# sleveque/control

Measured on AMD Instinct MI355X. Metric: Krylov iterations/s (preconditioned GMRES(10), all-at-once heat-control KKT), higher is better.
Workload: dtype f64; 1 GPU; 2-D heat control, 256^2 P1, n_t=64, beta=0.0001, T=2, BE, mode G; unknowns=8454272, krylov=gmres, left preconditioning, restart 10, classical Gram-Schmidt, parallelism=time-block rows over 1 GPU(s), transport=none, sweep_tiles=boxes from the dof coordinates (kkt_set_tile_coordinates)

## Files before the change

control_amd/_lib.py:

```python
from __future__ import annotations

import ctypes as C
import os

import numpy as np

_HERE = os.path.dirname(os.path.abspath(__file__))
LIB_PATH = os.environ.get("KKT_LIB") or os.path.join(_HERE, "libkkt.so")

c_i32p = C.POINTER(C.c_int32)
c_f64p = C.POINTER(C.c_double)


class KktError(RuntimeError):
    def __init__(self, code, msg):
        super().__init__(f"libkkt error {code}: {msg}")
        self.code = code


class PcDesc(C.Structure):
    _fields_ = [("kind", C.c_int), ("n_t", C.c_int), ("tau", C.c_double),
                ("beta", C.c_double), ("epsilon", C.c_double), ("nx", C.c_int64),
                ("m_indptr", c_i32p), ("m_indices", c_i32p), ("m_values", c_f64p),
                ("n_bc", C.c_int64), ("bc_idx", c_i32p),
# ... 54 lines not shown
    def as_dict(self):
        return {n: getattr(self, n) for n, _ in self._fields_}


class CoarseStats(C.Structure):
    _fields_ = ([(n, C.c_int64) for n in ("matrices", "launches", "n_coarse")] + [("ms", C.c_double)]
                + [(n, C.c_int64) for n in ("blocks", "block_n")])

    def as_dict(self):
        return {n: getattr(self, n) for n, _ in self._fields_}


class SpectrumStats(C.Structure):
    _fields_ = ([(n, C.c_int64) for n in ("matrices", "batches", "lanczos_steps", "power_steps", "launches",
                                          "syncs", "twin_syncs", "lanczos_syncs_max", "fallbacks",
                                          "batch_bytes")] + [("ms", C.c_double)])

    def as_dict(self):
        return {n: getattr(self, n) for n, _ in self._fields_}


class StepLock(C.Structure):
    _fields_ = [("n_steps", C.c_int), ("restart", C.c_int), ("V", c_f64p), ("h", c_f64p),
                ("v_next", c_f64p)]


class RelinDesc(C.Structure):
    _fields_ = ([("n_t", C.c_int), ("cn", C.c_int), ("nq", C.c_int),
                 ("ne", C.c_int64), ("n2", C.c_int64), ("n1", C.c_int64),
                 ("nu", C.c_double), ("tau", C.c_double), ("beta", C.c_double),
                 ("V", c_i32p)] + [(n, c_f64p) for n in ("W", "phi", "gphi", "lam", "glam")]
# ... 186 lines not shown
    "kkt_debug_coarse_inverses": (C.c_int, [C.c_void_p, c_f64p, C.c_int64]),
    "kkt_debug_dense_inverse": (C.c_int, [C.c_void_p, C.c_int, C.c_int, c_f64p, c_f64p, c_i32p]),
    "kkt_debug_coarse_correction": (C.c_int, [C.c_void_p, C.c_int, C.c_int, C.c_int64, c_f64p, c_f64p,
                                              c_f64p, c_f64p, c_f64p, c_f64p, c_i32p]),
    "kkt_debug_krylov_op": (C.c_int, [C.c_void_p, C.c_int, C.c_int64, C.c_int, c_f64p, c_f64p,
                                      c_f64p, C.c_double, C.c_double, c_f64p, c_f64p, c_f64p]),
    "kkt_debug_block_op": (C.c_int, [C.c_void_p, C.POINTER(BlockOp)]),
    "kkt_debug_spectrum_op": (C.c_int, [C.c_void_p, C.POINTER(SpectrumOp)]),
    "kkt_debug_row_step": (C.c_int, [C.c_void_p, C.POINTER(RowStep)]),
    "kkt_debug_tile_levels": (C.c_int, [C.c_void_p, C.POINTER(TileLevels)]),
    "kkt_debug_set_steplock": (C.c_int, [C.c_void_p, C.POINTER(StepLock)]),
    "kkt_debug_apply_forms": (C.c_int, [C.c_void_p, c_i32p, C.c_int]),
    "kkt_debug_pc_forms": (C.c_int, [C.c_void_p, c_i32p, C.c_int]),
    "kkt_debug_pc_solves": (C.c_int, [C.c_void_p, c_f64p, C.c_int]),
    "kkt_debug_pc_matrices": (C.c_int, [C.c_void_p, c_f64p, C.c_int]),
    "kkt_debug_mass_tile_values": (C.c_int, [C.c_void_p, C.POINTER(C.c_int64), C.POINTER(C.c_int64),
                                             c_f64p, c_i32p, c_f64p]),
    "kkt_get_info": (C.c_int, [C.c_void_p, C.POINTER(Info)]),
    "kkt_comm_unique_id": (C.c_int, [C.c_void_p]),
    "kkt_comm_init_rccl": (C.c_int, [C.c_void_p, C.c_void_p]),
    "kkt_comm_init_callbacks": (C.c_int, [C.c_void_p, ALLREDUCE_FN, SENDRECV_FN,
                                          C.c_void_p]),
    "kkt_comm_barrier": (C.c_int, [C.c_void_p]),
    "kkt_comm_max": (C.c_int, [C.c_void_p, c_f64p]),
}

_lib = None


def load():
# ... 25 lines not shown
```

control_amd/csrc/capi.cpp:

```cpp
#include <algorithm>
#include <charconv>
#include <climits>
#include <cmath>
#include <cstring>
#include <string>

#include "comm.hpp"
#include "pc.hpp"
#include "reaction.hpp"
#include "relin.hpp"
#include "system.hpp"
#include "tiles.hpp"

using namespace kkt;

struct kkt_system {
    System S;
};

static std::string g_create_error;

#define KKT_TRY(h, ...)                                   \
    if (!(h)) return KKT_ERR_ARG;                         \
    System &S = (h)->S;                                   \
// ... 74 lines not shown
    {"no_graph", "0 | 1", set_switch<&Options::no_graph>},
    {"persistent", "0 | 1", set_switch<&Options::persistent>},
    {"prog_mode", "auto | tile | dataflow | flags | w", set_prog_mode},
    {"prog_waves", "1..8", set_int<&Options::prog_waves, 1, 8>},
    {"prog_steps", "0 | 1", set_switch<&Options::prog_steps>},
    {"tile_depth", "1..16", set_int<&Options::tile_depth, 1, TILE_MAX_DEPTH>},
    {"tile_waves", "1..16", set_int<&Options::tile_waves, 1, 16>},
    {"tile_unfused", "0 | 1", set_switch<&Options::tile_unfused>},
    {"tile_poll_delay", "an integer", set_int<&Options::tile_poll_delay>},
    {"lanes", "0 | 1", set_switch<&Options::lanes>},
    {"lane_chunks", "an integer", set_int<&Options::lane_chunks>},
    {"coarse_setup", "batched | columns", set_coarse_setup},
    {"coarse_keep", "0 | 1", set_switch<&Options::coarse_keep>},
    {"coarse_blocks", "0 | 1", set_switch<&Options::coarse_blocks>},
    {"spectrum_batch", "0..4096", set_int<&Options::spectrum_batch, 0, 4096>},
    {"coarse_rings", "0 | 1", set_switch<&Options::coarse_rings>},
    {"tile_coarse_cache", "auto | 0 | 1 | 2", set_tile_coarse_cache},
    {"tile_coarse_rows", "block | full", set_tile_coarse_rows},
    {"mass_tiles", "0 | 1", set_switch<&Options::mass_tiles>},
    {"mass_tile_depth", "0..8", set_int<&Options::mass_tile_depth, 0, MASS_TILE_MAX_DEPTH>},
    {"mass_tile_rows", "0..65536", set_int<&Options::mass_tile_rows, 0, 65536>},
    {"mass_tile_levels", "0..4096", set_int<&Options::mass_tile_levels, 0, 4096>},
    {"mass_tile_waves", "0 | 4 | 8", set_mass_tile_waves},
    {"stage_timers", "0 | 1", set_switch<&Options::stage_timers>},
    {"verbose", "0 | 1", set_switch<&Options::verbose>},
    {"stamps", "0 | 1", set_switch<&Options::stamps>},
    {"debug_drop_handoff", "an integer", set_int<&Options::debug_drop_handoff>},
};

extern "C" {
// ... 481 lines not shown
            const bool grouped = L.ngroups > 0 && rowops_grouped_kernel(L.R, L.uniform_w);
            rec.insert(rec.end(), {L.R, L.uniform_w, grouped ? L.ngroups : 0, sorted});
        }
        return put_forms(rec, KKT_APPLY_FORM_INTS, out, cap);
    });
}

int kkt_debug_pc_forms(kkt_handle h, int32_t *out, int cap) {
    KKT_TRY(h, {
        std::vector<int32_t> rec;
        if (S.pc) S.pc->plain_forms(rec);
        return put_forms(rec, KKT_PC_FORM_INTS, out, cap);
    });
}

static int put_records(const std::vector<double> &rec, int per, double *out, int cap) {
    const int n = (int)rec.size() / per;
    if (out) {
        if (cap < (int)rec.size()) fail(KKT_ERR_ARG, "buffer too small for the records");
        std::copy(rec.begin(), rec.end(), out);
    }
    return n;
}

int kkt_debug_pc_solves(kkt_handle h, double *out, int cap) {
    KKT_TRY(h, {
        std::vector<double> rec;
        if (S.pc) S.pc->solve_records(rec);
        return put_records(rec, KKT_PC_SOLVE_VALS, out, cap);
    });
// ... 71 lines not shown
```

control_amd/csrc/pc.cpp:

```cpp
#include "pc.hpp"

#include <algorithm>
#include <chrono>
#include <cmath>
#include <cstdlib>
#include <cstdio>
#include <cstring>

namespace kkt {

SchurPC::SchurPC(System &S, const kkt_pc_desc &d) : S_(S), d_(d) {
    if (!S.finalized) fail(KKT_ERR_STATE, "kkt_set_pc_schur needs a finalized system");
    if (d.kind < KKT_PC_STATIONARY || d.kind > KKT_PC_INSTATIONARY_CN)
        fail(KKT_ERR_ARG, "unknown preconditioner kind");
    if (!d.m_indptr || !d.m_indices || !d.m_values) fail(KKT_ERR_ARG, "mass matrix missing");
    if (S.nx0 != S.nx1 || d.nx != S.nx0)
        fail(KKT_ERR_ARG, "built-in preconditioner needs equal spatial spaces of size nx");
    nx_ = d.nx;
    if (d.kind == KKT_PC_STATIONARY)
        n_ = 1;
    else
        n_ = d.kind == KKT_PC_INSTATIONARY_BE ? d.n_t : d.n_t - 1;
    if (n_ != S.n0 || n_ != S.n1 || n_ < 1)
        fail(KKT_ERR_ARG, "n_t does not match the block counts of the system");
// ... 63 lines not shown

void SchurPC::emit_wait(int lane, int ev) {
    PcStep s;
    s.kind = PcStep::EV_WAIT;
    s.lane = lane;
    s.ev = ev;
    steps_.push_back(s);
}

void SchurPC::values_changed() {
    clear_program();
    values_mem_.release();
    mats_.clear();
    mat_recs_.clear();
    solve_recs_.clear();
    einvs_.clear();
    pending_coarse_.clear();
    S_.spectrum_stats = kkt_spectrum_stats{};
    collect_matrices();
    if (d_.kind == KKT_PC_STATIONARY)
        build_stationary();
    else if (d_.kind == KKT_PC_INSTATIONARY_BE)
        build_BE();
    else
        build_CN();
    pre_.clear();
    pre_cls_.clear();
    flush_coarse();
    if (S_.opts.verbose && d_.schur_emin <= 0) {
        std::fprintf(stderr, "[kkt] Chebyshev sub-solves: degree %d; %lld Lanczos steps spent on "
// ... 400 lines not shown
        return out;
    }
    const bool be = d_.kind == KKT_PC_INSTATIONARY_BE;
    const double shift = d_.tau / std::sqrt(d_.beta);
    auto coef = [&](int i) {
        if (!be) return 0.5 * d_.tau / std::sqrt(d_.beta);
        return i == 0 ? 0.0 : (i == n - 1 ? std::sqrt(d_.epsilon) * shift : shift);
    };
    const int imid = (lo + hi) / 2;
    out.emplace_back(block_vals(KKT_Q10, imid, imid), coef(imid));
    for (int i = lo; i < hi; ++i) out.emplace_back(block_vals(KKT_Q10, i, i), coef(i));
    for (int i = hi - 1; i >= lo; --i) out.emplace_back(block_vals(KKT_Q01, i, i), coef(i));
    return out;
}

void SchurPC::collect_matrices() {
    pre_.clear();
    pre_cls_.clear();
    const int nbatch = S_.opts.spectrum_batch;
    const bool estimates = d_.schur_emin <= 0;
    if (nbatch <= 0 || !(estimates || coarse_cycles_ > 0)) return;
    const Pattern &P = S_.patterns[m_pat_];
    hipStream_t st = S_.stream;
    kkt_spectrum_stats &stats = S_.spectrum_stats;
    SpectrumCounters cnt;
    HIPCHK(hipStreamSynchronize(st));
    const auto t0 = std::chrono::steady_clock::now();
    std::vector<MatKey> keys;
    for (const auto &bc : solved_matrices()) {
        uint64_t bits;
        std::memcpy(&bits, &bc.second, sizeof bits);
        const MatKey key(bc.first, bits);
        if (pre_.count(key)) continue;
        Pre pr;
        pr.vals = values_mem_.alloc<double>(P.npadded);
        pr.dinv = values_mem_.alloc<double>(nx_);
        form_matrix(bc.first, bc.second, pr.vals, pr.dinv);
        cnt.launches += mask_ ? 3 : 2;
        pre_[key] = pr;
        keys.push_back(key);
    }
    const int C = (int)keys.size();
    if (C == 0) return;
    spec::TwinGroups twins;
    twins.first_of.resize(C);
    for (int i = 0; i < C; ++i) twins.first_of[i] = i;
    twins.pair_of.assign(C, -1);
    std::vector<unsigned> h_flag;
    DevPool tmp;
    if (C > 1) {
        std::vector<const double *> h_vals(C);
        for (int i = 0; i < C; ++i) h_vals[i] = pre_[keys[i]].vals;
        const double *const *d_vals = tmp.upload(h_vals.data(), h_vals.size());
        const int nw = spec_fingerprint_blocks(P.npadded);
        unsigned long long *d_fp = tmp.alloc<unsigned long long>((size_t)C * nw);
        std::vector<unsigned long long> h_fp((size_t)C * nw);
        launch_spec_fingerprint(st, d_vals, C, P.npadded, d_fp);
        HIPCHK(hipGetLastError());
        HIPCHK(hipMemcpyAsync(h_fp.data(), d_fp, h_fp.size() * sizeof(unsigned long long),
                              hipMemcpyDeviceToHost, st));
        HIPCHK(hipStreamSynchronize(st));
        cnt.launches++;
        cnt.syncs++;
        stats.twin_syncs++;
        std::vector<uint64_t> shifts(C), folded(C);
        for (int i = 0; i < C; ++i) {
            shifts[i] = keys[i].second;
            folded[i] = spec_fingerprint_fold(&h_fp[(size_t)i * nw], nw);
        }
        twins = spec::group_twins(shifts, folded);
        std::vector<SpecPair> pairs;
        for (const auto &pr : twins.pairs) pairs.push_back(SpecPair{h_vals[pr.first], h_vals[pr.second]});
        if (!pairs.empty()) {
            const SpecPair *d_pairs = tmp.upload(pairs.data(), pairs.size());
            unsigned *d_flag = tmp.alloc<unsigned>(pairs.size());
            h_flag.assign(pairs.size(), 1u);
            HIPCHK(hipMemsetAsync(d_flag, 0, pairs.size() * sizeof(unsigned), st));
            launch_spec_pairs_differ(st, d_pairs, (int)pairs.size(), P.npadded, d_flag);
            HIPCHK(hipGetLastError());
            HIPCHK(hipMemcpyAsync(h_flag.data(), d_flag, h_flag.size() * sizeof(unsigned),
                                  hipMemcpyDeviceToHost, st));
            HIPCHK(hipStreamSynchronize(st));
            cnt.launches++;
            cnt.syncs++;
            stats.twin_syncs++;
        }
    }
    std::vector<int> reps;
    const std::vector<int> cls = spec::twin_classes(twins, h_flag, &reps);
    for (int i = 0; i < C; ++i) pre_[keys[i]].cls = cls[i];
    pre_cls_.assign(reps.size(), PreCls{});
    const int32_t *tpos = estimates ? transpose_positions() : nullptr;
    for (size_t r0 = 0; estimates && r0 < reps.size(); r0 += (size_t)nbatch) {
        const int B = (int)std::min<size_t>((size_t)nbatch, reps.size() - r0);
        DevPool bmem;
        std::vector<const double *> lv(B), dv(B);
        std::vector<SpecSplit> split(B);
        std::vector<unsigned> nonsym(B, 0u);
        for (int b = 0; b < B; ++b) {
            const Pre &pr = pre_[keys[reps[r0 + b]]];
            lv[b] = pr.vals;
            dv[b] = pr.dinv;
        }
        size_t split_bytes = 0;
        if (tpos) {
            for (int b = 0; b < B; ++b)
// ... 59 lines not shown
    std::memcpy(&bits, &c, sizeof bits);
    auto key = std::make_pair(base_vals, bits);
    auto it = mats_.find(key);
    if (it != mats_.end() && (!solved || it->second.est != KKT_PC_EST_NONE)) return it->second;
    const Pattern &P = S_.patterns[m_pat_];
    hipStream_t st = S_.stream;
    Mat m;
    if (it != mats_.end()) {
        m = it->second;
    } else {
        const auto pre = pre_.find(key);
        if (pre != pre_.end()) {
            m.vals = pre->second.vals;
            m.dinv = pre->second.dinv;
        } else {
            m.vals = values_mem_.alloc<double>(P.npadded);
            m.dinv = values_mem_.alloc<double>(nx_);
            form_matrix(base_vals, c, m.vals, m.dinv);
        }
        m.index = (int)mat_recs_.size();
        MatRec r;
        r.c = c;
        mat_recs_.push_back(r);
    }
    if (!solved) {
        mats_[key] = m;
        return m;
    }
    MatRec &rec = mat_recs_[m.index];
    const Mat *twin = nullptr;
    kkt_spectrum_stats &stats = S_.spectrum_stats;
    const bool batched = S_.opts.spectrum_batch > 0;
    auto cls_of = [&](const MatKey &k) {
// ... 15 lines not shown
            fell_back = batched;
            stats.launches++;
            stats.syncs++;
            stats.twin_syncs++;
            auto d_flag = DevBuf<unsigned>::alloc(1);
            HIPCHK(hipMemsetAsync(d_flag.get(), 0, sizeof(unsigned), st));
            launch_vals_differ(st, m.vals, kv.second.vals, P.npadded, d_flag.get());
            unsigned differ = 1;
            HIPCHK(hipMemcpyAsync(&differ, d_flag.get(), sizeof differ, hipMemcpyDeviceToHost, st));
            HIPCHK(hipStreamSynchronize(st));
            if (!differ) {
                twin = &kv.second;
                break;
            }
        }
    }
    if (d_.schur_emin > 0) {
        m.emin = d_.schur_emin;
        m.emax = d_.schur_emax;
        m.eimag = d_.schur_eimag > 0 ? d_.schur_eimag : 0.0;
        m.est = KKT_PC_EST_GIVEN;
    } else if (twin) {
        m.emin = twin->emin;
        m.emax = twin->emax;
        m.eimag = twin->eimag;
        m.est = KKT_PC_EST_SHARED;
    } else {
        DevBuf<double> hv, sv2;
        unsigned nonsym = 0;
        Spectrum sp{0.0, 0.0, 0};
// ... 38 lines not shown
            rec.power = power;
        }
        if (coarse_cycles_ > 0) m.emin = std::max(m.emin, m.emax / 30.0);
        m.est = KKT_PC_EST_LANCZOS;
    }
    if (fell_back) stats.fallbacks++;
    if (!batched || fell_back)
        stats.ms += std::chrono::duration<double, std::milli>(std::chrono::steady_clock::now() - t0).count();
    if (coarse_cycles_ > 0) m.einv = twin && twin->einv ? twin->einv : coarse_inverse(m.vals);
    rec.est = m.est;
    rec.coarse = m.einv != nullptr;
    mats_[key] = m;
    return m;
}

void SchurPC::note_solve(int sweep, int level, const Mat &m) {
    mat_recs_[m.index].solves++;
    solve_recs_.insert(solve_recs_.end(),
                       {(double)sweep, (double)level, (double)m.index, mat_recs_[m.index].c, m.emin,
                        m.emax, m.eimag, (double)schur_its_, (double)m.est});
}

void SchurPC::solve_records(std::vector<double> &out) const { out = solve_recs_; }
bool SchurPC::coarse_space(CoarseDev *c, GalerkinDev *g, int64_t *n) const {
    if (coarse_.nc <= 0) return false;
    *c = coarse_;
    *g = galerkin_;
    *n = nx_;
    return true;
}

// ... 192 lines not shown
    if (record_solo) {
        solo.its = its;
        solo.lev = level_form(nullptr, sv[0], scale).lev;
        solo.eligible = true;
        end_level(std::move(solo));
    }
}

void SchurPC::build_stationary() {
    const double c = 1.0 / std::sqrt(d_.beta);
    const double *Dv = block_vals(KKT_Q10, 0, 0);
    const double *Dz = block_vals(KKT_Q01, 0, 0);
    double *b0 = in_, *b1 = in_ + nx_;
    double *u0 = out_, *u1 = out_ + nx_;
    emit_solves({Solve{m_vals_, m_dinv_, b0, u0}}, d_.mass_its, d_.mass_emin, d_.mass_emax, P_, nx_);
    emit_lin({Lin{{Term{Dv, u0}}, B_, 1.0, 0.0, -1.0, nullptr, b1}});
    Mat S1 = schur_matrix(Dv, c), S2 = schur_matrix(Dz, c);
    schur_its_ = resolve_its(S1);
    note_solve(KKT_PC_SWEEP_FIRST, 0, S1);
    emit_solves({Solve{S1.vals, S1.dinv, B_, u1}}, schur_its_, S1.emin, S1.emax, P_, nx_, false, nullptr, S1.eimag, &S1);
    emit_lin({Lin{{Term{m_vals_, u1}}, B_, 1.0}});
    note_solve(KKT_PC_SWEEP_SECOND, 0, S2);
    emit_solves({Solve{S2.vals, S2.dinv, B_, u1}}, schur_its_, S2.emin, S2.emax, P_, nx_, false, nullptr, S2.eimag, &S2);
}


void SchurPC::build_BE() {
    const int n = n_, lo = lo_, hi = hi_;
    const double tau = d_.tau, eps = d_.epsilon;
    const double shift = tau / std::sqrt(d_.beta);
    const int64_t nl = hi - lo;
// ... 16 lines not shown
        const int c0 = cfirst[c], c1 = cfirst[c + 1];
        cur_lane_ = lanes ? 1 : 0;
        {
            std::vector<Solve> sv;
            for (int i = c0; i < c1; ++i)
                sv.push_back(Solve{m_vals_, m_dinv_, blk(b0, i), blk(u0, i), 1.0 / tau,
                                   i == n - 1 ? 1.0 / eps : 1.0});
            double *const Pc[3] = {blk(P_[0], c0), blk(P_[1], c0), blk(P_[2], c0)};
            emit_solves(sv, d_.mass_its, d_.mass_emin, d_.mass_emax, Pc, nx_);
        }
        if (c == n_chunks - 1 && (up >= 0 || dn >= 0)) emit_comm(blk(u0, hi - 1), up, h_u0_, dn);
        {
            std::vector<Lin> ops;
            for (int i = c0; i < c1; ++i) {
                Lin l;
                l.terms.push_back(Term{block_vals(KKT_Q10, i, i), blk(u0, i)});
                if (i >= 1)
                    l.terms.push_back(Term{block_vals(KKT_Q10, i, i - 1),
                                           i - 1 >= lo ? blk(u0, i - 1) : h_u0_});
                l.y = blk(B_, i);
                l.cz = -1.0;
                l.z = blk(b1, i);
                ops.push_back(l);
            }
            emit_lin(ops);
        }
        if (lanes) chunk_done[c] = emit_record(1);
        cur_lane_ = 0;
    };
    auto sweep_chunk = [&](int c) {
        if (lanes) emit_wait(0, chunk_done[c]);
        for (int i = cfirst[c]; i < cfirst[c + 1]; ++i) {
            Mat F = schur_matrix(block_vals(KKT_Q10, i, i), coef(i));
            note_solve(KKT_PC_SWEEP_FORWARD, i, F);
            const Solve sv{F.vals, F.dinv, blk(B_, i), blk(u1, i)};
            if (i >= 1)
                emit_update_and_solve(Lin{{Term{block_vals(KKT_Q10, i, i - 1),
                                                i - 1 >= lo ? blk(u1, i - 1) : h_u1_}},
                                          blk(B_, i), -1.0, 1.0, 0.0, blk(B_, i), nullptr},
                                      sv, schur_its_, F.emin, F.emax, F.eimag, &F);
            else
                emit_solves({sv}, schur_its_, F.emin, F.emax, P_, nx_, false, nullptr, F.eimag, &F);
        }
    };
    if (lanes) {
        const int e_start = emit_record(0);
        emit_wait(1, e_start);
        side_chunk(0);
        for (int c = 0; c < n_chunks; ++c) {
            sweep_chunk(c);
            if (c + 1 < n_chunks) side_chunk(c + 1);
        }
    } else {
        side_chunk(0);
        if (dn >= 0) emit_comm(nullptr, -1, h_u1_, dn);
        sweep_chunk(0);
    }
    if (up >= 0) emit_comm(blk(u1, hi - 1), up, nullptr, -1);
    {
        std::vector<Lin> ops;
        for (int i = lo; i < hi; ++i)
            ops.push_back(Lin{{Term{m_vals_, blk(u1, i)}}, blk(B_, i),
                              i == n - 1 ? eps * tau : tau});
        emit_lin(ops);
    }
    if (up >= 0) emit_comm(nullptr, -1, h_u1_, up);
    for (int i = hi - 1; i >= lo; --i) {
        Mat G = schur_matrix(block_vals(KKT_Q01, i, i), coef(i));
        note_solve(KKT_PC_SWEEP_BACKWARD, i, G);
        const Solve sv{G.vals, G.dinv, blk(B_, i), blk(u1, i)};
        if (i <= n - 2)
            emit_update_and_solve(Lin{{Term{block_vals(KKT_Q01, i, i + 1),
                                            i + 1 < hi ? blk(u1, i + 1) : h_u1_}},
                                      blk(B_, i), -1.0, 1.0, 0.0, blk(B_, i), nullptr},
                                  sv, schur_its_, G.emin, G.emax, G.eimag, &G);
        else
            emit_solves({sv}, schur_its_, G.emin, G.emax, P_, nx_, false, nullptr, G.eimag, &G);
    }
    if (dn >= 0) emit_comm(blk(u1, lo), dn, nullptr, -1);
}

void SchurPC::build_CN() {
    const int n = n_, lo = lo_, hi = hi_;
    const double tau = d_.tau;
    const double c = 0.5 * tau / std::sqrt(d_.beta);
    const int64_t nl = hi - lo;
    const int nloc = (int)nl;
    double *b0 = in_, *b1 = in_ + nl * nx_;
// ... 9 lines not shown
    emit_time(T_, b0, 3, nloc, nullptr, up >= 0 ? h_t_ : nullptr);
    if (dn >= 0) emit_comm(blk(T_, lo), dn, nullptr, -1);
    {
        std::vector<Solve> sv;
        for (int i = lo; i < hi; ++i)
            sv.push_back(Solve{m_vals_, m_dinv_, blk(T_, i), blk(u0, i), 2.0 / tau, 1.0});
        emit_solves(sv, d_.mass_its, d_.mass_emin, d_.mass_emax, P_, nx_);
    }
    if (dn >= 0) emit_comm(nullptr, -1, h_u0_, dn);
    emit_time(u0, u0, 4, nloc, dn >= 0 ? h_u0_ : nullptr, nullptr);
    if (up >= 0) emit_comm(blk(u0, hi - 1), up, nullptr, -1);
    {
        std::vector<Lin> ops;
        for (int i = lo; i < hi; ++i) {
            Lin l;
            l.terms.push_back(Term{block_vals(KKT_Q10, i, i), blk(u0, i)});
            if (i >= 1)
                l.terms.push_back(Term{block_vals(KKT_Q10, i, i - 1),
                                       i - 1 >= lo ? blk(u0, i - 1) : h_u0_});
            l.y = blk(B_, i);
            ops.push_back(l);
        }
        emit_lin(ops);
    }
    if (up >= 0 || dn >= 0) emit_comm(blk(B_, hi - 1), up, h_t_, dn);
    emit_time(B_, B_, 2, nloc, dn >= 0 ? h_t_ : nullptr, nullptr);
    {
        std::vector<Lin> ops;
        for (int i = lo; i < hi; ++i)
            ops.push_back(Lin{{}, blk(B_, i), 0.0, 1.0, -1.0, blk(B_, i), blk(b1, i)});
        emit_lin(ops);
    }
    if (dn >= 0) emit_comm(nullptr, -1, h_t_, dn);
    emit_time(B_, B_, 4, nloc, dn >= 0 ? h_t_ : nullptr, nullptr);
    if (up >= 0) emit_comm(blk(B_, hi - 1), up, nullptr, -1);
    if (dn >= 0) emit_comm(nullptr, -1, h_u1_, dn);
    for (int i = lo; i < hi; ++i) {
        Mat F = schur_matrix(block_vals(KKT_Q10, i, i), c);
        note_solve(KKT_PC_SWEEP_FORWARD, i, F);
        const Solve sv{F.vals, F.dinv, blk(B_, i), blk(u1, i)};
        if (i >= 1) {
            const double *prev = i - 1 >= lo ? blk(u1, i - 1) : h_u1_;
            emit_update_and_solve(Lin{{Term{block_vals(KKT_Q10, i, i - 1), prev},
                                       Term{cM.vals, prev}},
                                      blk(B_, i), -1.0, 1.0, 0.0, blk(B_, i), nullptr},
                                  sv, schur_its_, F.emin, F.emax, F.eimag, &F);
        } else {
            emit_solves({sv}, schur_its_, F.emin, F.emax, P_, nx_, false, nullptr, F.eimag, &F);
        }
    }
    if (up >= 0) emit_comm(blk(u1, hi - 1), up, nullptr, -1);
    emit_time(u1, u1, 2, nloc, dn >= 0 ? h_u1_ : nullptr, nullptr);
    {
        std::vector<Lin> ops;
        for (int i = lo; i < hi; ++i)
            ops.push_back(Lin{{Term{m_vals_, blk(u1, i)}}, blk(B_, i), 0.5 * tau});
        emit_lin(ops);
    }
    if (up >= 0) emit_comm(nullptr, -1, h_u1_, up);
    for (int i = hi - 1; i >= lo; --i) {
        Mat G = schur_matrix(block_vals(KKT_Q01, i, i), c);
        note_solve(KKT_PC_SWEEP_BACKWARD, i, G);
        const Solve sv{G.vals, G.dinv, blk(B_, i), blk(u1, i)};
        if (i <= n - 2) {
            Mat H = schur_matrix(block_vals(KKT_Q01, i, i + 1), c, false);
            emit_update_and_solve(Lin{{Term{H.vals, i + 1 < hi ? blk(u1, i + 1) : h_u1_}},
                                      blk(B_, i), -1.0, 1.0, 0.0, blk(B_, i), nullptr},
                                  sv, schur_its_, G.emin, G.emax, G.eimag, &G);
        } else {
            emit_solves({sv}, schur_its_, G.emin, G.emax, P_, nx_, false, nullptr, G.eimag, &G);
        }
    }
    if (dn >= 0) emit_comm(blk(u1, lo), dn, nullptr, -1);
}

void SchurPC::emit_comm(const double *send, int dst, double *recv, int src) {
    PcStep s;
    s.kind = PcStep::COMM;
    s.x = send;
    s.y = recv;
// ... 140 lines not shown
```

control_amd/csrc/pc.hpp:

```cpp
#pragma once
#include <map>
#include <string>
#include <vector>

#include "comm.hpp"
#include "rowlaunch.hpp"
#include "spectrum_host.hpp"
#include "system.hpp"
#include "tiles.hpp"

namespace kkt {

Spectrum jacobi_spectrum(System &S, int pattern, const double *vals, const double *dinv,
                         const uint8_t *rowmask, int max_steps,
                         bool zero_mean = false);
double jacobi_skew_radius(System &S, int pattern, const double *skew_vals, const double *dinv,
                          const uint8_t *rowmask, int max_steps, int *steps_out);

struct SpectrumCounters {
    int64_t launches = 0, syncs = 0, lanczos_syncs_max = 0, bytes = 0;
};
std::vector<Spectrum> jacobi_spectrum_batch(System &S, int pattern, const std::vector<const double *> &vals,
                                            const std::vector<const double *> &dinv, const uint8_t *rowmask,
                                            int max_steps, SpectrumCounters *cnt);
// ... 57 lines not shown
    virtual double *in() = 0;
    virtual double *out() = 0;
    virtual void values_changed() {}
    virtual void check() {}
    virtual bool timed_out(std::string *) { return false; }
    virtual bool fallback_plain() { return false; }
    virtual const unsigned *err_word() const { return nullptr; }
    virtual void time_stages(kkt_pc_stage_times *out);
    virtual void debug_read(unsigned long long *, int) {}
    virtual void plain_forms(std::vector<int32_t> &) const {}
    virtual void mass_tile_debug(int64_t *, int64_t *, double *, int32_t *, double *) {
        fail(KKT_ERR_STATE, "kkt_debug_mass_tile_values: no mass solves on tiles on this handle");
    }
    virtual void solve_records(std::vector<double> &) const {}
    virtual void matrix_records(std::vector<double> &) const {}
    virtual bool coarse_space(CoarseDev *, GalerkinDev *, int64_t *) const { return false; }
    virtual void debug_tile_levels(kkt_tile_levels *) {
        fail(KKT_ERR_STATE, "kkt_debug_tile_levels: no two-grid tile program on this handle");
    }
    virtual void time_programs(float *ms, int *launches, int64_t *phases) {
        *ms = 0.f;
        *launches = 0;
        *phases = 0;
    }
};

class SchurPC : public PcBase {
   public:
    SchurPC(System &S, const kkt_pc_desc &d);
    void run() override;
// ... 1 lines not shown
    double *out() override { return out_; }
    void values_changed() override;
    void check() override;
    bool timed_out(std::string *why) override;
    bool fallback_plain() override;
    const unsigned *err_word() const override { return d_err_; }
    void time_stages(kkt_pc_stage_times *out) override;
    void debug_read(unsigned long long *out, int n) override;
    void plain_forms(std::vector<int32_t> &out) const override;
    void mass_tile_debug(int64_t *n_entries, int64_t *n_vals, double *copy, int32_t *gpos,
                         double *vals) override;
    void solve_records(std::vector<double> &out) const override;
    bool coarse_space(CoarseDev *c, GalerkinDev *g, int64_t *n) const override;
    void debug_tile_levels(kkt_tile_levels *run) override;
    void matrix_records(std::vector<double> &out) const override;
    void time_programs(float *ms, int *launches, int64_t *phases) override;
    int bc_set() const { return bc_set_; }
    int schur_its() const { return schur_its_; }
    int coarse_cycles() const { return coarse_cycles_; }
    double typical_emin() const { return typical_emin_; }
    double typical_emax() const { return typical_emax_; }
    int64_t n_launches() const { return (int64_t)steps_.size(); }

   private:
    System &S_;
    kkt_pc_desc d_;
    Stream side_;
    std::vector<Event> events_;
    DevPool handle_mem_, values_mem_, program_mem_;
    std::vector<int32_t> m_indptr_, m_indices_, bc_idx_;
// ... 13 lines not shown
        double *vals;
        double *dinv;
        double emin = 0.0, emax = 0.0;
        double eimag = 0.0;
        double *einv = nullptr;
        int index = -1;
        int est = KKT_PC_EST_NONE;
    };
    struct MatRec {
        double c = 0.0;
        int est = KKT_PC_EST_NONE, lanczos = 0, power = 0, solves = 0;
        bool coarse = false;
    };
    std::vector<MatRec> mat_recs_;
    std::vector<double> solve_recs_;
    void note_solve(int sweep, int level, const Mat &m);
    int schur_its_ = 0;
    double typical_emin_ = 0.0, typical_emax_ = 0.0;
    int resolve_its(const Mat &typical);
    int64_t spectrum_steps_ = 0;
    int coarse_cycles_ = 0;
    std::vector<int32_t> p_indptr_, p_indices_;
    std::vector<double> p_values_;
    std::vector<int32_t> pt_indptr_, pt_indices_;
    std::vector<double> pt_values_;
    CoarseDev coarse_;
    std::vector<const double *> einvs_;
    double *R_ = nullptr;
    void build_coarse();
    GalerkinDev galerkin_{};
    double *coarse_inverse(const double *vals);
// ... 23 lines not shown
    Mat schur_matrix(const double *base_vals, double c, bool solved = true);
    using MatKey = std::pair<const double *, uint64_t>;
    struct Pre {
        double *vals = nullptr, *dinv = nullptr;
        int cls = -1;
    };
    struct PreCls {
        bool estimated = false;
        Spectrum sp{0.0, 0.0, 0};
        bool nonsym = false;
        double radius = 0.0;
        int power = 0;
    };
    std::map<MatKey, Pre> pre_;
    std::vector<PreCls> pre_cls_;
    void form_matrix(const double *base_vals, double c, double *vals, double *dinv);
    std::vector<std::pair<const double *, double>> solved_matrices() const;
    void collect_matrices();
    void emit_lin(const std::vector<Lin> &ops);
    void emit_cheb(const std::vector<Cheb> &ops);
    double *il_P_[3] = {nullptr, nullptr, nullptr};
    size_t il_cap_ = 0;
    void emit_time(double *y, const double *x, int kind, int n, const double *lo_halo = nullptr,
                   const double *hi_halo = nullptr);
    void emit_comm(const double *send, int dst, double *recv, int src);
    struct Solve {
        const double *vals, *dinv, *b;
        double *out;
        double post1 = 1.0, post2 = 1.0;
    };
// ... 150 lines not shown
```

control_amd/csrc/spectrum_host.hpp:

```cpp
#pragma once
#include <algorithm>
#include <cmath>
#include <cstdint>
#include <map>
#include <utility>
#include <vector>

#if defined(__HIPCC__)
#define KKT_SPEC_HD __host__ __device__ inline
#else
#define KKT_SPEC_HD inline
#endif

namespace kkt {

struct Spectrum {
    double emin, emax;
    int steps;
};

namespace spec {

constexpr int RITZ_FIRST = 30, RITZ_EVERY = 10;
constexpr int POWER_MIN_STEPS = 8;
// ... 129 lines not shown
    }
    bool any_active() const {
        for (uint32_t a : active)
            if (a) return true;
        return false;
    }
    Spectrum result(int b) const { return ritz_result(alpha[b], beta[b]); }
};

struct TwinGroups {
    std::vector<int> first_of;
    std::vector<std::pair<int, int>> pairs;
    std::vector<int> pair_of;
};
inline TwinGroups group_twins(const std::vector<uint64_t> &shift_bits,
                              const std::vector<uint64_t> &fingerprint) {
    const int C = (int)shift_bits.size();
    TwinGroups T;
    T.first_of.resize(C);
    T.pair_of.assign(C, -1);
    std::map<std::pair<uint64_t, uint64_t>, int> groups;
    for (int i = 0; i < C; ++i) {
        T.first_of[i] = i;
        const auto g = std::make_pair(shift_bits[i], fingerprint[i]);
        const auto it = groups.find(g);
        if (it == groups.end()) {
            groups[g] = i;
            continue;
        }
        T.first_of[i] = it->second;
        T.pair_of[i] = (int)T.pairs.size();
        T.pairs.emplace_back(it->second, i);
    }
    return T;
}
inline std::vector<int> twin_classes(TwinGroups &T, const std::vector<unsigned> &differ,
                                     std::vector<int> *reps) {
    const int C = (int)T.first_of.size();
    for (int i = 0; i < C; ++i)
// ... 17 lines not shown
```

control_amd/csrc/system.hpp:

```cpp
#pragma once
#include <hip/hip_runtime_api.h>
#include <stdint.h>

#include <map>
#include <memory>
#include <string>
#include <tuple>
#include <vector>

#include "../../include/kkt.h"
#include "devmem.hpp"
#include "kernels.hpp"

namespace kkt {

struct Error {
    int code;
    std::string msg;
};
[[noreturn]] void fail(int code, const std::string &msg);
enum class ProgMode { Auto, Tile, Dataflow, Flags, W };
struct Options {
    int sell_r = 2, sell_sigma = 8;
    bool sell_sort = true, shared_rows = true, ragged_switch = true;
    bool ragged_xcd = true, apply_xcd = false, pc_xcd = true;
    bool interleave = true, kernarg_ops = false, no_graph = false, lanes = false;
    int lane_chunks = 4;
    bool persistent = true, prog_steps = true, tile_unfused = false;
    ProgMode prog_mode = ProgMode::Auto;
    int prog_waves = 0, tile_depth = 0, tile_waves = 0;
    bool coarse_columns = false;
    bool coarse_keep = false, coarse_blocks = true;
    int spectrum_batch = 32;
    bool coarse_rings = true;
    int tile_coarse_cache = -1;
    bool tile_coarse_full = false;
    bool mass_tiles = true;
    int mass_tile_depth = 0, mass_tile_rows = 0, mass_tile_levels = 0, mass_tile_waves = 0;
    bool stage_timers = false, verbose = false, stamps = false;
    int tile_poll_delay = 24, debug_drop_handoff = 0;
};

struct Pattern {
    int64_t nrows = 0, ncols = 0, nnz = 0;
    int R = 2;
    int nslices = 0;
    int64_t nslots = 0;
    int64_t npadded = 0;
// ... 243 lines not shown
```

control_amd/multiblock.py:

```python
from __future__ import annotations

import ctypes as C
import os
from dataclasses import dataclass
from typing import Optional, Sequence

import numpy as np

from . import _lib

__all__ = ["Nullspace", "NoneNullspace", "ConstantNullspace", "DirichletBCNullspace",
           "FullNullspace", "MultiBlockSystem", "SchurPC", "StokesPC", "KSPResult",
           "ChebSpec", "PatternOnly"]

Q00, Q01, Q10, Q11 = 0, 1, 2, 3
_KSP_TYPES = {"gmres": 0, "fgmres": 1, "minres": 2}
_PC_SIDES = {"left": 0, "right": 1, 0: 0, 1: 1}


class Nullspace:
    """``preconditioner.py:75-116`` (the corrections themselves run on the device)."""


class NoneNullspace(Nullspace):
# ... 296 lines not shown
        n = fn(self._h, None, 0)
        if n < 0:
            self._ck(n)
        rec = np.zeros(n * len(fields), dtype=np.int32)
        got = fn(self._h, rec.ctypes.data_as(_lib.c_i32p), rec.size)
        if got < 0:
            self._ck(got)
        return [dict(zip(fields, map(int, r))) for r in rec.reshape(n, len(fields))]

    def apply_forms(self):
        return self._forms(self._lib.kkt_debug_apply_forms, ("R", "uniform_w", "groups", "sorted"))

    def pc_forms(self):
        return self._forms(self._lib.kkt_debug_pc_forms,
                           ("form", "width", "slots", "lane", "count", "variant"))

    def _records(self, fn, width):
        n = fn(self._h, None, 0)
        if n < 0:
            self._ck(n)
        rec = np.zeros(n * width)
        got = fn(self._h, rec.ctypes.data_as(_lib.c_f64p), rec.size)
        if got < 0:
            self._ck(got)
        return rec.reshape(n, width)

    _SWEEPS = ("first", "second", "forward", "backward", "kp")
    _ESTIMATES = ("given", "lanczos", "shared", "none", "zero_mean", "upper")

    def pc_solves(self):
# ... 314 lines not shown
```

include/kkt.h:

```cpp
#ifndef KKT_H
#define KKT_H

#include <stdint.h>

#ifdef __cplusplus
extern "C" {
#endif

typedef struct kkt_system *kkt_handle;

enum {
    KKT_OK = 0,
    KKT_ERR_ARG = -1,
    KKT_ERR_HIP = -2,
    KKT_ERR_STATE = -3,
    KKT_ERR_CALLBACK = -4,
    KKT_ERR_COMM = -5
};

enum { KKT_Q00 = 0, KKT_Q01 = 1, KKT_Q10 = 2, KKT_Q11 = 3 };

enum { KKT_KSP_GMRES = 0, KKT_KSP_FGMRES = 1, KKT_KSP_MINRES = 2 };
enum { KKT_PC_SIDE_DEFAULT = -1, KKT_PC_LEFT = 0, KKT_PC_RIGHT = 1 };

// ... 214 lines not shown
    int64_t sweep_launches, sweep_phases, batched_launches, comm_steps;
} kkt_pc_stage_times;
int kkt_time_pc_stages(kkt_handle h, const double *d_x, double *d_y, kkt_pc_stage_times *out);

typedef struct kkt_coarse_stats {
    int64_t matrices, launches, n_coarse;
    double ms;
    int64_t blocks, block_n;
} kkt_coarse_stats;
int kkt_coarse_setup_stats(kkt_handle h, kkt_coarse_stats *out);

typedef struct kkt_spectrum_stats {
    int64_t matrices, batches, lanczos_steps, power_steps, launches, syncs, twin_syncs,
        lanczos_syncs_max, fallbacks, batch_bytes;
    double ms;
} kkt_spectrum_stats;
int kkt_spectrum_stats_get(kkt_handle h, kkt_spectrum_stats *out);
int kkt_debug_coarse_matrices(kkt_handle h, double *out, int64_t cap);
int kkt_debug_coarse_inverses(kkt_handle h, double *out, int64_t cap);
int kkt_debug_dense_inverse(kkt_handle h, int n, int nmat, const double *a, double *inv, int *bad);
#define KKT_COARSE_SHAPE_INTS 8
int kkt_debug_coarse_correction(kkt_handle h, int batched, int nb, int64_t vstride, const double *r,
                                const double *x_in, const double *einv, double *rc, double *ec,
                                double *x_out, int32_t *shape);

enum { KKT_KRYLOV_MDOT = 0, KKT_KRYLOV_ORTHOGONALISE = 1, KKT_KRYLOV_BUILD_SOLUTION = 2,
       KKT_KRYLOV_SCALE_INV = 3, KKT_KRYLOV_AXPBY = 4, KKT_KRYLOV_COPY = 5, KKT_KRYLOV_FILL = 6,
       KKT_KRYLOV_NORM2 = 7, KKT_KRYLOV_MAXPY = 8 };
#define KKT_KRYLOV_PAD (-6.02214076e23)
int kkt_debug_krylov_op(kkt_handle h, int op, int64_t n, int nv, const double *w, const double *V,
// ... 98 lines not shown
int kkt_debug_set_steplock(kkt_handle h, const kkt_steplock *lock);

enum { KKT_APPLY_FORM_INTS = 4, KKT_PC_FORM_INTS = 6 };
enum { KKT_PC_ROWS_PLAIN = 0, KKT_PC_ROWS_SHARED = 1, KKT_PC_ROWS_KERNARG = 2,
       KKT_PC_ROWS_INTERLEAVED = 3, KKT_PC_PROGRAM = 4, KKT_PC_TILE = 5, KKT_PC_TILE_CHEB = 6 };
int kkt_debug_apply_forms(kkt_handle h, int32_t *out, int cap);
int kkt_debug_pc_forms(kkt_handle h, int32_t *out, int cap);

enum { KKT_PC_SOLVE_VALS = 9, KKT_PC_MATRIX_VALS = 6 };
enum { KKT_PC_SWEEP_FIRST = 0, KKT_PC_SWEEP_SECOND = 1, KKT_PC_SWEEP_FORWARD = 2,
       KKT_PC_SWEEP_BACKWARD = 3, KKT_PC_SWEEP_KP = 4 };
enum { KKT_PC_EST_GIVEN = 0, KKT_PC_EST_LANCZOS = 1, KKT_PC_EST_SHARED = 2, KKT_PC_EST_NONE = 3,
       KKT_PC_EST_ZERO_MEAN = 4, KKT_PC_EST_UPPER = 5 };
int kkt_debug_pc_solves(kkt_handle h, double *out, int cap);
int kkt_debug_pc_matrices(kkt_handle h, double *out, int cap);

int kkt_debug_mass_tile_values(kkt_handle h, int64_t *n_entries, int64_t *n_vals, double *copy,
                               int32_t *gpos, double *vals);

typedef struct kkt_info {
    int64_t n_local;
    int64_t n_blocks_stored;
    int64_t n_value_arrays;
    int64_t n_patterns;
    int64_t nnz_blocks;
    int64_t rows_blocks;
    int64_t bytes_algorithmic;
    int64_t bytes_device_values;
    int64_t bytes_device_index;
    int64_t bytes_streamed;
// ... 33 lines not shown
```

Before: 173.2 Krylov iterations/s.

## Alias identical preconditioner block matrices so sweeps reuse one device copy

Adds a pc_alias option, on by default, that fingerprints the Schur-complement matrices and the off-diagonal coupling blocks used in the time sweeps. Identical ones collapse onto one representative device buffer, and the forward and backward sweeps then multiply and solve against that shared copy. The aim is to cut the distinct value arrays streamed per preconditioner apply, so repeated blocks can stay in cache, and to avoid forming duplicate matrices. The risk is a false match in the fingerprint, plus extra setup work and host syncs.

```diff
diff --git a/control_amd/_lib.py b/control_amd/_lib.py
--- a/control_amd/_lib.py
+++ b/control_amd/_lib.py
@@ -92,7 +92,8 @@
 class SpectrumStats(C.Structure):
     _fields_ = ([(n, C.c_int64) for n in ("matrices", "batches", "lanczos_steps", "power_steps", "launches",
                                           "syncs", "twin_syncs", "lanczos_syncs_max", "fallbacks",
-                                          "batch_bytes")] + [("ms", C.c_double)])
+                                          "batch_bytes")] + [("ms", C.c_double)] +
+                [(n, C.c_int64) for n in ("alias_blocks", "aliased")])
 
     def as_dict(self):
         return {n: getattr(self, n) for n, _ in self._fields_}
@@ -309,6 +310,7 @@
     "kkt_debug_pc_forms": (C.c_int, [C.c_void_p, c_i32p, C.c_int]),
     "kkt_debug_pc_solves": (C.c_int, [C.c_void_p, c_f64p, C.c_int]),
     "kkt_debug_pc_matrices": (C.c_int, [C.c_void_p, c_f64p, C.c_int]),
+    "kkt_debug_pc_alias": (C.c_int, [C.c_void_p, c_i32p, C.c_int]),
     "kkt_debug_mass_tile_values": (C.c_int, [C.c_void_p, C.POINTER(C.c_int64), C.POINTER(C.c_int64),
                                              c_f64p, c_i32p, c_f64p]),
     "kkt_get_info": (C.c_int, [C.c_void_p, C.POINTER(Info)]),
diff --git a/control_amd/csrc/capi.cpp b/control_amd/csrc/capi.cpp
--- a/control_amd/csrc/capi.cpp
+++ b/control_amd/csrc/capi.cpp
@@ -112,6 +112,7 @@
     {"coarse_keep", "0 | 1", set_switch<&Options::coarse_keep>},
     {"coarse_blocks", "0 | 1", set_switch<&Options::coarse_blocks>},
     {"spectrum_batch", "0..4096", set_int<&Options::spectrum_batch, 0, 4096>},
+    {"pc_alias", "0 | 1", set_switch<&Options::pc_alias>},
     {"coarse_rings", "0 | 1", set_switch<&Options::coarse_rings>},
     {"tile_coarse_cache", "auto | 0 | 1 | 2", set_tile_coarse_cache},
     {"tile_coarse_rows", "block | full", set_tile_coarse_rows},
@@ -623,6 +624,14 @@
     });
 }
 
+int kkt_debug_pc_alias(kkt_handle h, int32_t *out, int cap) {
+    KKT_TRY(h, {
+        std::vector<int32_t> rec;
+        if (S.pc) S.pc->alias_records(rec);
+        return put_forms(rec, KKT_PC_ALIAS_INTS, out, cap);
+    });
+}
+
 static int put_records(const std::vector<double> &rec, int per, double *out, int cap) {
     const int n = (int)rec.size() / per;
     if (out) {
diff --git a/control_amd/csrc/pc.cpp b/control_amd/csrc/pc.cpp
--- a/control_amd/csrc/pc.cpp
+++ b/control_amd/csrc/pc.cpp
@@ -101,6 +101,7 @@
     mats_.clear();
     mat_recs_.clear();
     solve_recs_.clear();
+    alias_recs_.clear();
     einvs_.clear();
     pending_coarse_.clear();
     S_.spectrum_stats = kkt_spectrum_stats{};
@@ -531,11 +532,34 @@
     return out;
 }
 
+std::vector<const double *> SchurPC::multiplied_blocks() const {
+    std::vector<const double *> out;
+    if (d_.kind == KKT_PC_STATIONARY) {
+        out.push_back(block_vals(KKT_Q10, 0, 0));
+        return out;
+    }
+    for (int i = lo_; i < hi_; ++i) {
+        out.push_back(block_vals(KKT_Q10, i, i));
+        if (i >= 1) out.push_back(block_vals(KKT_Q10, i, i - 1));
+    }
+    for (int i = hi_ - 1; i >= lo_; --i)
+        if (i <= n_ - 2) out.push_back(block_vals(KKT_Q01, i, i + 1));
+    return out;
+}
+
+const double *SchurPC::shared_block(const double *vals) const {
+    const auto it = block_rep_.find(vals);
+    return it == block_rep_.end() ? vals : it->second;
+}
+
 void SchurPC::collect_matrices() {
     pre_.clear();
     pre_cls_.clear();
+    block_rep_.clear();
+    formed_.clear();
     const int nbatch = S_.opts.spectrum_batch;
     const bool estimates = d_.schur_emin <= 0;
+    const bool alias = S_.opts.pc_alias;
     if (nbatch <= 0 || !(estimates || coarse_cycles_ > 0)) return;
     const Pattern &P = S_.patterns[m_pat_];
     hipStream_t st = S_.stream;
@@ -544,14 +568,17 @@
     HIPCHK(hipStreamSynchronize(st));
     const auto t0 = std::chrono::steady_clock::now();
     std::vector<MatKey> keys;
+    std::vector<DevBuf<double>> own_vals, own_dinv;
     for (const auto &bc : solved_matrices()) {
         uint64_t bits;
         std::memcpy(&bits, &bc.second, sizeof bits);
         const MatKey key(bc.first, bits);
         if (pre_.count(key)) continue;
+        own_vals.push_back(DevBuf<double>::alloc(P.npadded));
+        own_dinv.push_back(DevBuf<double>::alloc(nx_));
         Pre pr;
-        pr.vals = values_mem_.alloc<double>(P.npadded);
-        pr.dinv = values_mem_.alloc<double>(nx_);
+        pr.vals = own_vals.back().get();
+        pr.dinv = own_dinv.back().get();
         form_matrix(bc.first, bc.second, pr.vals, pr.dinv);
         cnt.launches += mask_ ? 3 : 2;
         pre_[key] = pr;
@@ -559,20 +586,25 @@
     }
     const int C = (int)keys.size();
     if (C == 0) return;
+    std::vector<const double *> h_vals(C);
+    for (int i = 0; i < C; ++i) h_vals[i] = pre_[keys[i]].vals;
+    if (alias)
+        for (const double *b : multiplied_blocks())
+            if (std::find(h_vals.begin() + C, h_vals.end(), b) == h_vals.end()) h_vals.push_back(b);
+    const int N = (int)h_vals.size();
+    stats.alias_blocks += N - C;
     spec::TwinGroups twins;
-    twins.first_of.resize(C);
-    for (int i = 0; i < C; ++i) twins.first_of[i] = i;
-    twins.pair_of.assign(C, -1);
+    twins.first_of.resize(N);
+    for (int i = 0; i < N; ++i) twins.first_of[i] = i;
+    twins.pair_of.assign(N, -1);
     std::vector<unsigned> h_flag;
     DevPool tmp;
-    if (C > 1) {
-        std::vector<const double *> h_vals(C);
-        for (int i = 0; i < C; ++i) h_vals[i] = pre_[keys[i]].vals;
+    if (N > 1) {
         const double *const *d_vals = tmp.upload(h_vals.data(), h_vals.size());
         const int nw = spec_fingerprint_blocks(P.npadded);
-        unsigned long long *d_fp = tmp.alloc<unsigned long long>((size_t)C * nw);
-        std::vector<unsigned long long> h_fp((size_t)C * nw);
-        launch_spec_fingerprint(st, d_vals, C, P.npadded, d_fp);
+        unsigned long long *d_fp = tmp.alloc<unsigned long long>((size_t)N * nw);
+        std::vector<unsigned long long> h_fp((size_t)N * nw);
+        launch_spec_fingerprint(st, d_vals, N, P.npadded, d_fp);
         HIPCHK(hipGetLastError());
         HIPCHK(hipMemcpyAsync(h_fp.data(), d_fp, h_fp.size() * sizeof(unsigned long long),
                               hipMemcpyDeviceToHost, st));
@@ -580,12 +612,13 @@
         cnt.launches++;
         cnt.syncs++;
         stats.twin_syncs++;
-        std::vector<uint64_t> shifts(C), folded(C);
-        for (int i = 0; i < C; ++i) {
-            shifts[i] = keys[i].second;
+        std::vector<uint64_t> shifts(N, 0), folded(N);
+        std::vector<int> tag(N, 1);
+        for (int i = 0; i < N; ++i) {
+            if (i < C) shifts[i] = keys[i].second, tag[i] = 0;
             folded[i] = spec_fingerprint_fold(&h_fp[(size_t)i * nw], nw);
         }
-        twins = spec::group_twins(shifts, folded);
+        twins = spec::group_twins(shifts, folded, tag);
         std::vector<SpecPair> pairs;
         for (const auto &pr : twins.pairs) pairs.push_back(SpecPair{h_vals[pr.first], h_vals[pr.second]});
         if (!pairs.empty()) {
@@ -603,10 +636,31 @@
             stats.twin_syncs++;
         }
     }
+    std::vector<int> all_reps;
+    const std::vector<int> cls = spec::twin_classes(twins, h_flag, &all_reps);
+    for (int i = 0; i < C; ++i) pre_[keys[i]].cls = cls[i];
+    pre_cls_.assign(all_reps.size(), PreCls{});
+    for (int i = 0; i < N; ++i) {
+        const int first = alias && cls[i] >= 0 ? all_reps[cls[i]] : i;
+        if (first != i) stats.aliased++;
+        if (i >= C) {
+            if (first != i) block_rep_[h_vals[i]] = h_vals[first];
+            continue;
+        }
+        Pre &pr = pre_[keys[i]];
+        if (first != i) {
+            pr.vals = pre_[keys[first]].vals;
+            pr.dinv = pre_[keys[first]].dinv;
+            own_vals[i].reset();
+            own_dinv[i].reset();
+        } else {
+            values_mem_.adopt(std::move(own_vals[i]));
+            values_mem_.adopt(std::move(own_dinv[i]));
+        }
+    }
     std::vector<int> reps;
-    const std::vector<int> cls = spec::twin_classes(twins, h_flag, &reps);
-    for (int i = 0; i < C; ++i) pre_[keys[i]].cls = cls[i];
-    pre_cls_.assign(reps.size(), PreCls{});
+    for (int r : all_reps)
+        if (r < C) reps.push_back(r);
     const int32_t *tpos = estimates ? transpose_positions() : nullptr;
     for (size_t r0 = 0; estimates && r0 < reps.size(); r0 += (size_t)nbatch) {
         const int B = (int)std::min<size_t>((size_t)nbatch, reps.size() - r0);
@@ -696,9 +750,16 @@
             m.vals = pre->second.vals;
             m.dinv = pre->second.dinv;
         } else {
-            m.vals = values_mem_.alloc<double>(P.npadded);
-            m.dinv = values_mem_.alloc<double>(nx_);
-            form_matrix(base_vals, c, m.vals, m.dinv);
+            auto &f = formed_[MatKey(shared_block(base_vals), bits)];
+            if (!f.first) {
+                f.first = values_mem_.alloc<double>(P.npadded);
+                f.second = values_mem_.alloc<double>(nx_);
+                form_matrix(base_vals, c, f.first, f.second);
+            } else {
+                S_.spectrum_stats.aliased++;
+            }
+            m.vals = f.first;
+            m.dinv = f.second;
         }
         m.index = (int)mat_recs_.size();
         MatRec r;
@@ -744,6 +805,11 @@
                 break;
             }
         }
+    }
+    if (twin && S_.opts.pc_alias && m.vals != twin->vals) {
+        m.vals = twin->vals;
+        m.dinv = twin->dinv;
+        stats.aliased++;
     }
     if (d_.schur_emin > 0) {
         m.emin = d_.schur_emin;
@@ -812,7 +878,20 @@
     return m;
 }
 
-void SchurPC::note_solve(int sweep, int level, const Mat &m) {
+void SchurPC::alias_records(std::vector<int32_t> &out) const {
+    out.clear();
+    std::map<const double *, int32_t> number;
+    for (const double *p : alias_recs_) {
+        if (p && !number.count(p)) {
+            const int32_t k = (int32_t)number.size();
+            number[p] = k;
+        }
+        out.push_back(p ? number[p] : -1);
+    }
+}
+
+void SchurPC::note_solve(int sweep, int level, const Mat &m, const double *upd_vals) {
+    alias_recs_.insert(alias_recs_.end(), {m.vals, m.dinv, upd_vals});
     mat_recs_[m.index].solves++;
     solve_recs_.insert(solve_recs_.end(),
                        {(double)sweep, (double)level, (double)m.index, mat_recs_[m.index].c, m.emin,
@@ -1035,7 +1114,7 @@
     double *b0 = in_, *b1 = in_ + nx_;
     double *u0 = out_, *u1 = out_ + nx_;
     emit_solves({Solve{m_vals_, m_dinv_, b0, u0}}, d_.mass_its, d_.mass_emin, d_.mass_emax, P_, nx_);
-    emit_lin({Lin{{Term{Dv, u0}}, B_, 1.0, 0.0, -1.0, nullptr, b1}});
+    emit_lin({Lin{{Term{shared_block(Dv), u0}}, B_, 1.0, 0.0, -1.0, nullptr, b1}});
     Mat S1 = schur_matrix(Dv, c), S2 = schur_matrix(Dz, c);
     schur_its_ = resolve_its(S1);
     note_solve(KKT_PC_SWEEP_FIRST, 0, S1);
@@ -1082,9 +1161,9 @@
             std::vector<Lin> ops;
             for (int i = c0; i < c1; ++i) {
                 Lin l;
-                l.terms.push_back(Term{block_vals(KKT_Q10, i, i), blk(u0, i)});
+                l.terms.push_back(Term{mult_vals(KKT_Q10, i, i), blk(u0, i)});
                 if (i >= 1)
-                    l.terms.push_back(Term{block_vals(KKT_Q10, i, i - 1),
+                    l.terms.push_back(Term{mult_vals(KKT_Q10, i, i - 1),
                                            i - 1 >= lo ? blk(u0, i - 1) : h_u0_});
                 l.y = blk(B_, i);
                 l.cz = -1.0;
@@ -1100,11 +1179,11 @@
         if (lanes) emit_wait(0, chunk_done[c]);
         for (int i = cfirst[c]; i < cfirst[c + 1]; ++i) {
             Mat F = schur_matrix(block_vals(KKT_Q10, i, i), coef(i));
-            note_solve(KKT_PC_SWEEP_FORWARD, i, F);
+            const double *upd = i >= 1 ? mult_vals(KKT_Q10, i, i - 1) : nullptr;
+            note_solve(KKT_PC_SWEEP_FORWARD, i, F, upd);
             const Solve sv{F.vals, F.dinv, blk(B_, i), blk(u1, i)};
             if (i >= 1)
-                emit_update_and_solve(Lin{{Term{block_vals(KKT_Q10, i, i - 1),
-                                                i - 1 >= lo ? blk(u1, i - 1) : h_u1_}},
+                emit_update_and_solve(Lin{{Term{upd, i - 1 >= lo ? blk(u1, i - 1) : h_u1_}},
                                           blk(B_, i), -1.0, 1.0, 0.0, blk(B_, i), nullptr},
                                       sv, schur_its_, F.emin, F.emax, F.eimag, &F);
             else
@@ -1135,11 +1214,11 @@
     if (up >= 0) emit_comm(nullptr, -1, h_u1_, up);
     for (int i = hi - 1; i >= lo; --i) {
         Mat G = schur_matrix(block_vals(KKT_Q01, i, i), coef(i));
-        note_solve(KKT_PC_SWEEP_BACKWARD, i, G);
+        const double *upd = i <= n - 2 ? mult_vals(KKT_Q01, i, i + 1) : nullptr;
+        note_solve(KKT_PC_SWEEP_BACKWARD, i, G, upd);
         const Solve sv{G.vals, G.dinv, blk(B_, i), blk(u1, i)};
         if (i <= n - 2)
-            emit_update_and_solve(Lin{{Term{block_vals(KKT_Q01, i, i + 1),
-                                            i + 1 < hi ? blk(u1, i + 1) : h_u1_}},
+            emit_update_and_solve(Lin{{Term{upd, i + 1 < hi ? blk(u1, i + 1) : h_u1_}},
                                       blk(B_, i), -1.0, 1.0, 0.0, blk(B_, i), nullptr},
                                   sv, schur_its_, G.emin, G.emax, G.eimag, &G);
         else
@@ -1179,9 +1258,9 @@
         std::vector<Lin> ops;
         for (int i = lo; i < hi; ++i) {
             Lin l;
-            l.terms.push_back(Term{block_vals(KKT_Q10, i, i), blk(u0, i)});
+            l.terms.push_back(Term{mult_vals(KKT_Q10, i, i), blk(u0, i)});
             if (i >= 1)
-                l.terms.push_back(Term{block_vals(KKT_Q10, i, i - 1),
+                l.terms.push_back(Term{mult_vals(KKT_Q10, i, i - 1),
                                        i - 1 >= lo ? blk(u0, i - 1) : h_u0_});
             l.y = blk(B_, i);
             ops.push_back(l);
@@ -1202,11 +1281,12 @@
     if (dn >= 0) emit_comm(nullptr, -1, h_u1_, dn);
     for (int i = lo; i < hi; ++i) {
         Mat F = schur_matrix(block_vals(KKT_Q10, i, i), c);
-        note_solve(KKT_PC_SWEEP_FORWARD, i, F);
+        const double *upd = i >= 1 ? mult_vals(KKT_Q10, i, i - 1) : nullptr;
+        note_solve(KKT_PC_SWEEP_FORWARD, i, F, upd);
         const Solve sv{F.vals, F.dinv, blk(B_, i), blk(u1, i)};
         if (i >= 1) {
             const double *prev = i - 1 >= lo ? blk(u1, i - 1) : h_u1_;
-            emit_update_and_solve(Lin{{Term{block_vals(KKT_Q10, i, i - 1), prev},
+            emit_update_and_solve(Lin{{Term{upd, prev},
                                        Term{cM.vals, prev}},
                                       blk(B_, i), -1.0, 1.0, 0.0, blk(B_, i), nullptr},
                                   sv, schur_its_, F.emin, F.emax, F.eimag, &F);
@@ -1225,10 +1305,11 @@
     if (up >= 0) emit_comm(nullptr, -1, h_u1_, up);
     for (int i = hi - 1; i >= lo; --i) {
         Mat G = schur_matrix(block_vals(KKT_Q01, i, i), c);
-        note_solve(KKT_PC_SWEEP_BACKWARD, i, G);
+        Mat H{};
+        if (i <= n - 2) H = schur_matrix(block_vals(KKT_Q01, i, i + 1), c, false);
+        note_solve(KKT_PC_SWEEP_BACKWARD, i, G, H.vals);
         const Solve sv{G.vals, G.dinv, blk(B_, i), blk(u1, i)};
         if (i <= n - 2) {
-            Mat H = schur_matrix(block_vals(KKT_Q01, i, i + 1), c, false);
             emit_update_and_solve(Lin{{Term{H.vals, i + 1 < hi ? blk(u1, i + 1) : h_u1_}},
                                       blk(B_, i), -1.0, 1.0, 0.0, blk(B_, i), nullptr},
                                   sv, schur_its_, G.emin, G.emax, G.eimag, &G);
diff --git a/control_amd/csrc/pc.hpp b/control_amd/csrc/pc.hpp
--- a/control_amd/csrc/pc.hpp
+++ b/control_amd/csrc/pc.hpp
@@ -95,6 +95,7 @@
     }
     virtual void solve_records(std::vector<double> &) const {}
     virtual void matrix_records(std::vector<double> &) const {}
+    virtual void alias_records(std::vector<int32_t> &) const {}
     virtual bool coarse_space(CoarseDev *, GalerkinDev *, int64_t *) const { return false; }
     virtual void debug_tile_levels(kkt_tile_levels *) {
         fail(KKT_ERR_STATE, "kkt_debug_tile_levels: no two-grid tile program on this handle");
@@ -126,6 +127,7 @@
     bool coarse_space(CoarseDev *c, GalerkinDev *g, int64_t *n) const override;
     void debug_tile_levels(kkt_tile_levels *run) override;
     void matrix_records(std::vector<double> &out) const override;
+    void alias_records(std::vector<int32_t> &out) const override;
     void time_programs(float *ms, int *launches, int64_t *phases) override;
     int bc_set() const { return bc_set_; }
     int schur_its() const { return schur_its_; }
@@ -169,7 +171,8 @@
     };
     std::vector<MatRec> mat_recs_;
     std::vector<double> solve_recs_;
-    void note_solve(int sweep, int level, const Mat &m);
+    std::vector<const double *> alias_recs_;
+    void note_solve(int sweep, int level, const Mat &m, const double *upd_vals = nullptr);
     int schur_its_ = 0;
     double typical_emin_ = 0.0, typical_emax_ = 0.0;
     int resolve_its(const Mat &typical);
@@ -223,6 +226,11 @@
     };
     std::map<MatKey, Pre> pre_;
     std::vector<PreCls> pre_cls_;
+    std::map<const double *, const double *> block_rep_;
+    std::map<MatKey, std::pair<double *, double *>> formed_;
+    const double *shared_block(const double *vals) const;
+    std::vector<const double *> multiplied_blocks() const;
+    const double *mult_vals(int q, int i, int j) const { return shared_block(block_vals(q, i, j)); }
     void form_matrix(const double *base_vals, double c, double *vals, double *dinv);
     std::vector<std::pair<const double *, double>> solved_matrices() const;
     void collect_matrices();
diff --git a/control_amd/csrc/spectrum_host.hpp b/control_amd/csrc/spectrum_host.hpp
--- a/control_amd/csrc/spectrum_host.hpp
+++ b/control_amd/csrc/spectrum_host.hpp
@@ -167,15 +167,17 @@
     std::vector<int> pair_of;
 };
 inline TwinGroups group_twins(const std::vector<uint64_t> &shift_bits,
-                              const std::vector<uint64_t> &fingerprint) {
+                              const std::vector<uint64_t> &fingerprint,
+                              const std::vector<int> &tag = {}) {
     const int C = (int)shift_bits.size();
     TwinGroups T;
     T.first_of.resize(C);
     T.pair_of.assign(C, -1);
-    std::map<std::pair<uint64_t, uint64_t>, int> groups;
+    std::map<std::pair<int, std::pair<uint64_t, uint64_t>>, int> groups;
     for (int i = 0; i < C; ++i) {
         T.first_of[i] = i;
-        const auto g = std::make_pair(shift_bits[i], fingerprint[i]);
+        const auto g = std::make_pair(tag.empty() ? 0 : tag[i],
+                                      std::make_pair(shift_bits[i], fingerprint[i]));
         const auto it = groups.find(g);
         if (it == groups.end()) {
             groups[g] = i;
diff --git a/control_amd/csrc/system.hpp b/control_amd/csrc/system.hpp
--- a/control_amd/csrc/system.hpp
+++ b/control_amd/csrc/system.hpp
@@ -32,6 +32,7 @@
     bool coarse_columns = false;
     bool coarse_keep = false, coarse_blocks = true;
     int spectrum_batch = 32;
+    bool pc_alias = true;
     bool coarse_rings = true;
     int tile_coarse_cache = -1;
     bool tile_coarse_full = false;
diff --git a/control_amd/multiblock.py b/control_amd/multiblock.py
--- a/control_amd/multiblock.py
+++ b/control_amd/multiblock.py
@@ -334,6 +334,9 @@
     def pc_forms(self):
         return self._forms(self._lib.kkt_debug_pc_forms,
                            ("form", "width", "slots", "lane", "count", "variant"))
+
+    def pc_alias(self):
+        return self._forms(self._lib.kkt_debug_pc_alias, ("matrix", "dinv", "update"))
 
     def _records(self, fn, width):
         n = fn(self._h, None, 0)
diff --git a/include/kkt.h b/include/kkt.h
--- a/include/kkt.h
+++ b/include/kkt.h
@@ -252,6 +252,7 @@
     int64_t matrices, batches, lanczos_steps, power_steps, launches, syncs, twin_syncs,
         lanczos_syncs_max, fallbacks, batch_bytes;
     double ms;
+    int64_t alias_blocks, aliased;
 } kkt_spectrum_stats;
 int kkt_spectrum_stats_get(kkt_handle h, kkt_spectrum_stats *out);
 int kkt_debug_coarse_matrices(kkt_handle h, double *out, int64_t cap);
@@ -380,6 +381,8 @@
        KKT_PC_EST_ZERO_MEAN = 4, KKT_PC_EST_UPPER = 5 };
 int kkt_debug_pc_solves(kkt_handle h, double *out, int cap);
 int kkt_debug_pc_matrices(kkt_handle h, double *out, int cap);
+enum { KKT_PC_ALIAS_INTS = 3 };
+int kkt_debug_pc_alias(kkt_handle h, int32_t *out, int cap);
 
 int kkt_debug_mass_tile_values(kkt_handle h, int64_t *n_entries, int64_t *n_vals, double *copy,
                                int32_t *gpos, double *vals);
```

Result: faster. 181.2 Krylov iterations/s (median of 6 runs) (+4.6%).
